# HugoZHL/MEVI

Measured on AMD Instinct MI355X. Metric: queries/sec @ MRR@10-match, MSMARCO dev, 1/2/4/8 MI355X, higher is better.
Workload: dtype f16+f32; 1 GPU; C2 dense arm (faiss_search.py Flat): 6980 x 768 f32 queries x 8841823 x 768 f32 docs, exact inner-product top-1000; queries=6980, docs=8841823, dim=768, topk=1000, parallelism=single GPU

## Files before the change

mevi_amd/csrc/ip_topk.hip:

```cpp

#include "mfma_pp_f16x16.h"

#include <float.h>
#include <math.h>
#include <string.h>
#include <vector>

namespace mevi {
namespace {

constexpr int MAX_SORT = 16384;

struct TopkGeom {
  int k;
  int S;
  int cap;
};

static inline int next_pow2(int x) {
  int p = 1;
  while (p < x) p <<= 1;
  return p;
}

// ... 465 lines not shown
  }
  __syncthreads();
}

__global__ __launch_bounds__(256) void compact_kernel(unsigned long long *__restrict__ buf,
                                                     unsigned int *__restrict__ count,
                                                     float *__restrict__ tau,
                                                     unsigned int *__restrict__ failed, int nq, int S, int k,
                                                     int cap) {
  extern __shared__ __attribute__((aligned(16))) unsigned long long skeys[];
  unsigned int *hist = reinterpret_cast<unsigned int *>(skeys + S);
  for (int q = blockIdx.x; q < nq; q += gridDim.x)
    compact_query(skeys, hist, buf + (size_t)q * S, count, tau, failed, q, k, cap);
}

template <int KPL>
__global__ __launch_bounds__(256) void compact_wave_kernel(unsigned long long *__restrict__ buf, unsigned int *__restrict__ count,
                                                          float *__restrict__ tau, unsigned int *__restrict__ failed, int nq,
                                                          int S, int k, int cap) {
  const int lane = threadIdx.x & 63;
  const int q = blockIdx.x * 4 + (int)(threadIdx.x >> 6);
  if (q >= nq) return;
  const unsigned int c_raw = count[q];
  if (c_raw == 0u) return;
  const int c = c_raw > (unsigned int)cap ? cap : (int)c_raw;
  const int n = k + c;
  if (n > 64 * KPL) return;
  unsigned long long *row = buf + (size_t)q * S;
  unsigned long long key[KPL];
#pragma unroll
  for (int j = 0; j < KPL; ++j) key[j] = (64 * j + lane < n) ? row[64 * j + lane] : 0ull;
  const int nj = (n + 63) >> 6;
  unsigned long long T = 0ull;
  bool exact = false;
  for (int b = 63; b >= 0; --b) {
    const unsigned long long cand = T | (1ull << b);
    int cnt = 0;
#pragma unroll
    for (int jb = 0; jb < KPL / 8; ++jb)
      if (8 * jb < nj) {
#pragma unroll
        for (int jj = 0; jj < 8; ++jj) cnt += __popcll(__ballot(key[8 * jb + jj] >= cand));
      }
    if (cnt >= k) {
      T = cand;
      if (cnt == k) {
        exact = true;
        break;
      }
    }
  }
  if (exact) {
    unsigned long long mn = ~0ull;
#pragma unroll
    for (int jb = 0; jb < KPL / 8; ++jb)
      if (8 * jb < nj) {
#pragma unroll
        for (int jj = 0; jj < 8; ++jj) {
          const unsigned long long kk = key[8 * jb + jj];
          if (kk >= T && kk < mn) mn = kk;
        }
      }
#pragma unroll
    for (int off = 32; off > 0; off >>= 1) {
      const unsigned long long o = ((unsigned long long)(unsigned int)__shfl_xor((int)(mn >> 32), off) << 32) |
                                   (unsigned int)__shfl_xor((int)mn, off);
      mn = o < mn ? o : mn;
    }
    T = mn;
  }
  int base = 0;
#pragma unroll
  for (int jb = 0; jb < KPL / 8; ++jb)
    if (8 * jb < nj) {
#pragma unroll
      for (int jj = 0; jj < 8; ++jj) {
        const unsigned long long kk = key[8 * jb + jj];
        const bool pass = kk > T;
        const unsigned long long mask = __ballot(pass);
        if (pass)
          row[base + (int)__builtin_amdgcn_mbcnt_hi((unsigned int)(mask >> 32), __builtin_amdgcn_mbcnt_lo((unsigned int)mask, 0u))] = kk;
        base += __popcll(mask);
      }
    }
  for (int i = base + lane; i < k; i += 64) row[i] = (i == k - 1) ? T : 0ull;
  if (lane == 0) {
    tau[q] = (T != 0ull) ? key_score(T) : -INFINITY;
    count[q] = 0u;
    if (c_raw > (unsigned int)cap) failed[q] = 1u;
  }
}

template <int KPL>
__global__ __launch_bounds__(256) void rank_tau_kernel(const unsigned long long *__restrict__ buf, int nq, int S, int k, int rank,
                                                      float *__restrict__ tau, float *__restrict__ tau_s) {
  const int lane = threadIdx.x & 63;
  const int q = blockIdx.x * 4 + (int)(threadIdx.x >> 6);
  if (q >= nq) return;
  const unsigned long long *row = buf + (size_t)q * S;
  unsigned long long key[KPL];
#pragma unroll
  for (int j = 0; j < KPL; ++j) key[j] = (64 * j + lane < k) ? row[64 * j + lane] : 0ull;
  const int nj = (k + 63) >> 6;
  unsigned long long T = 0ull;
// ... 851 lines not shown
      acc[1][0][r] = -INFINITY;
    }
    emit_tile<1>(acc, tq, 0, doc_begin + blk * 256 + 32 * w8, doc_end, buf, count, S, k, cap, id_base, stash);
    if (!have_nxt) break;
    blk = blk_n;
    cur = nxt;
    blk_n += gridDim.x;
    have_nxt = blk_n < n_blocks;
    if (have_nxt) nxt = src_of(blk_n);
  }
  asm volatile("s_waitcnt vmcnt(0)" ::: "memory");
  stash_flush(stash, buf, count, S, k, cap);
}

constexpr int RS_LD = 36;
__global__ __launch_bounds__(256) void rescore_rows_kernel(const float *__restrict__ Q, const float *__restrict__ D,
                                                          int dim, unsigned long long *__restrict__ buf, int S,
                                                          int kp, int nq, unsigned int id_base,
                                                          const float *__restrict__ qnorm,
                                                          const float *__restrict__ qinv,
                                                          const double *__restrict__ qshift, float c1, float c2,
                                                          const unsigned int *__restrict__ dmax_bits,
                                                          const float *__restrict__ dnorm_c,
                                                          unsigned int *__restrict__ err_ratio_bits,
                                                          const float *__restrict__ qdelta, const float *__restrict__ qn16,
                                                          const float *__restrict__ acc_k, int upper_keys = 0) {
  __shared__ __attribute__((aligned(16))) float tiles[4][64 * RS_LD];
  const int lane = threadIdx.x & 63;
  const int wave = __builtin_amdgcn_readfirstlane(threadIdx.x >> 6);
  const int wpq = (kp + 63) / 64;
  const long long gw = (long long)blockIdx.x * 4 + wave;
  const int q = (int)(gw / wpq);
  if (q >= nq) return;
  const int c = (int)(gw - (long long)q * wpq) * 64 + lane;
  unsigned long long *row = buf + (size_t)q * S;
  unsigned long long key = (c < kp) ? row[c] : 0ull;
  if (acc_k && key != 0ull) {
    const unsigned int idc = key_id(key) - id_base;
    const double e_max = h1_err_bound(qdelta[q], qn16[q], (double)__uint_as_float(dmax_bits[0]), (double)__uint_as_float(dmax_bits[3]), c1) +
                         (double)qnorm[q] * (double)c2 * __uint_as_float(dmax_bits[1]);
    const double e_c = h1_err_bound(qdelta[q], qn16[q], (double)dnorm_c[idc], (double)__uint_as_float(dmax_bits[3]), c1) +
                       (double)qnorm[q] * (double)c2 * __uint_as_float(dmax_bits[1]);
    if ((double)key_score(key) * (double)qinv[q] + e_c < (double)acc_k[q] * (double)qinv[q] - e_max) {
      key = 0ull;
      if (c < kp) row[c] = 0ull;
    }
  }
  const bool valid = key != 0ull;
  const unsigned int my_id = valid ? key_id(key) - id_base : 0u;
  float *sd = tiles[wave];
  const float *src[8];
#pragma unroll
  for (int i = 0; i < 8; ++i) src[i] = D + (size_t)__shfl(my_id, (lane >> 3) + 8 * i) * dim + (lane & 7) * 4;
  const float *qr = Q + (size_t)q * dim;
  const int nslab = (dim + 31) / 32;
  float4 v[8];
  auto fetch = [&](int s) {
    const bool in = s * 32 + (lane & 7) * 4 < dim;
#pragma unroll
    for (int i = 0; i < 8; ++i) v[i] = in ? *reinterpret_cast<const float4 *>(src[i] + s * 32) : make_float4(0.f, 0.f, 0.f, 0.f);
  };
  fetch(0);
  float acc = 0.f;
  for (int s = 0; s < nslab; ++s) {
#pragma unroll
    for (int i = 0; i < 8; ++i) *reinterpret_cast<float4 *>(sd + ((lane >> 3) + 8 * i) * RS_LD + (lane & 7) * 4) = v[i];
    if (s + 1 < nslab) fetch(s + 1);
    __builtin_amdgcn_wave_barrier();
    const float *dr = sd + lane * RS_LD;
#pragma unroll
    for (int k4 = 0; k4 < 32; k4 += 4) {
      const float4 x = *reinterpret_cast<const float4 *>(dr + k4);
      const int kk = s * 32 + k4;
      const float4 qq = kk < dim ? *reinterpret_cast<const float4 *>(qr + kk) : make_float4(0.f, 0.f, 0.f, 0.f);
      acc = fmaf(qq.x, x.x, acc);
      acc = fmaf(qq.y, x.y, acc);
      acc = fmaf(qq.z, x.z, acc);
      acc = fmaf(qq.w, x.w, acc);
    }
    __builtin_amdgcn_wave_barrier();
  }
  if (c < kp) row[c] = valid ? make_key(acc, key_id(key)) : 0ull;
  if (err_ratio_bits) {
    float ratio = 0.f;
    if (valid) {
      const double den = h1_err_bound(qdelta[q], qn16[q], (double)dnorm_c[my_id], (double)__uint_as_float(dmax_bits[3]), c1) +
                         (double)qnorm[q] * (double)c2 * __uint_as_float(dmax_bits[1]);
      const double est = (double)key_score(key) * (double)qinv[q] + qshift[q];
      if (den > 0.0) ratio = (float)((upper_keys ? fmax((double)acc - est, 0.0) : fabs(est - (double)acc)) / den);
    }
#pragma unroll
    for (int off = 32; off > 0; off >>= 1) ratio = fmaxf(ratio, __shfl_xor(ratio, off));
    if (lane == 0 && ratio > 0.f) atomicMax(err_ratio_bits, __float_as_uint(ratio));
  }
}

__global__ __launch_bounds__(256) void rescore_finish_kernel(const unsigned long long *__restrict__ buf, int S, int k,
                                                            int kp, const float *__restrict__ tau,
                                                            const float *__restrict__ qnorm,
                                                            const float *__restrict__ qinv,
                                                            const double *__restrict__ qshift, float c1, float c2,
                                                            const unsigned int *__restrict__ dmax_bits,
                                                            unsigned int *__restrict__ failed,
                                                            unsigned long long *__restrict__ out_top, int out_ld,
                                                            const float *__restrict__ qdelta, const float *__restrict__ qn16) {
  extern __shared__ __attribute__((aligned(16))) unsigned long long skeys[];
  const int q = blockIdx.x, t = threadIdx.x;
  int P = 64;
  while (P < kp) P <<= 1;
  const unsigned long long *row = buf + (size_t)q * S;
  for (int i = t; i < P; i += 256) skeys[i] = (i < kp) ? row[i] : 0ull;
  __syncthreads();
  bitonic_sort_desc<256>(skeys, P, t);
  for (int i = t; i < k; i += 256) out_top[(size_t)q * out_ld + i] = skeys[i];
  if (t == 0) {
    bool ok = true;
    const float a_last = tau[q];
    const double eps = h1_err_bound(qdelta[q], qn16[q], (double)__uint_as_float(dmax_bits[0]), (double)__uint_as_float(dmax_bits[3]), c1) +
                       (double)qnorm[q] * (double)c2 * __uint_as_float(dmax_bits[1]);
    if (a_last > -INFINITY) {
      const unsigned long long kth = skeys[k - 1];
      ok = (kth != 0ull) && ((double)a_last * (double)qinv[q] + qshift[q] + eps < (double)key_score(kth));
    }
    if (!(eps < 1.0e38)) ok = false;
    if (!ok) failed[q] = 1u;
  }
}

__global__ __launch_bounds__(256) void count_candidates_kernel(const unsigned int *__restrict__ count, int nq, int cap,
                                                              unsigned long long *__restrict__ out) {
  const int q = blockIdx.x * 256 + threadIdx.x;
  const unsigned int c = q < nq ? count[q] : 0u;
  unsigned long long sum = c;
  unsigned int mx = c, over = c > (unsigned int)cap ? 1u : 0u;
#pragma unroll
  for (int off = 32; off > 0; off >>= 1) {
    sum += ((unsigned long long)(unsigned int)__shfl_xor((int)(sum >> 32), off) << 32) | (unsigned int)__shfl_xor((int)sum, off);
    mx = max(mx, (unsigned int)__shfl_xor((int)mx, off));
    over += (unsigned int)__shfl_xor((int)over, off);
  }
// ... 38 lines not shown

struct ExactWs {
  SearchState st, fb;
  float *qsub; int *fidx;
  char *spare;
};
static ExactWs carve_exact(Carver &c, int64_t nq, int64_t dim, const TopkGeom &g) {
  return {carve_state(c, nq, g), carve_state(c, nq, g), c.take<float>((size_t)nq * dim), c.take<int>(nq), c.take<char>(256)};
}

struct QuerySide {
  float *image;
  float *norm, *inv, *delta, *n16;
  double *shift;
  unsigned int *err_bits;
};
static QuerySide carve_query_side(Carver &c, int64_t nq, size_t image_bytes) {
  QuerySide s = {reinterpret_cast<float *>(c.take<char>(image_bytes)), c.take<float>(nq + 1), c.take<float>(nq + 1),
                 c.take<float>(nq + 1), c.take<float>(nq + 1), c.take<double>(nq), nullptr};
  if (s.norm) s.err_bits = reinterpret_cast<unsigned int *>(s.norm + nq);
  return s;
}

thread_local double g_growth = 0.0;
thread_local int g_profile = 0;
thread_local mevi_ip_topk_stats g_stats = {0, 0, 0, 0.0, 0.0, 0.0, 0.0, 0.0, 0, 0, 0, 0};
thread_local std::vector<hipEvent_t> g_events;
thread_local std::vector<long long> g_chunk_rows;

static void profile_mark(hipStream_t stream) {
  if (!g_profile) return;
  hipEvent_t e;
  if (hipEventCreate(&e) != hipSuccess) return;
  (void)hipEventRecord(e, stream);
  g_events.push_back(e);
// ... 11 lines not shown
  }
  g_chunk_rows.clear();
  for (hipEvent_t e : g_events) (void)hipEventDestroy(e);
  g_events.clear();
}

enum class PassKind { ExactF32, F16Image, I8Image };
struct PassArgs {
  PassKind kind;
  const float *Q; int64_t nq;
  const float *D; int64_t nd; int dim;
  TopkGeom g; uint32_t id_base; SearchState st;
  bool guaranteed;
  unsigned long long *cand = nullptr;
  const float *row_scale = nullptr, *qub = nullptr;
};

enum class FilterGrid { PerTile, PerCU, SmallStream };
struct FilterChoice {
  const void *fn;
  size_t lds;
  int qt, ni16;
  FilterGrid grid;
};

static bool choose_filter(PassKind kind, int64_t nq, int dim, FilterChoice &f) {
  const bool h1 = kind != PassKind::ExactF32;
  const int ni = 2;
  static const bool shape32_f = [] { const char *e = getenv("MEVI_IP_FILTER_MFMA"); return e && atoi(e) == 32; }();
  static const int qt_pin = [] { const char *e = getenv("MEVI_IP_FILTER_QT"); return e ? atoi(e) : 0; }();
// ... 92 lines not shown
  const bool sample_on = sample_mode == 1 || (sample_mode != 0 && nq <= 1024);
  double s_c = 0.0;
  int64_t n_sample = 0;
  bool sampled = false;
  if (sample_on && !guaranteed && g.k <= 4096 && g.k >= 32) {
    const double r = g.k / 2 < 16 ? 16.0 : (g.k / 2 > 96 ? 96.0 : (double)(g.k / 2));
    double c = r >= 96.0 ? 3.0 : 8.0;
    const double c_fit = (double)g.cap / ((double)g.k * (1.0 + 8.0 / sqrt(r)));
    if (c_fit < c) c = c_fit;
    if (c >= 1.5 && (1.0 - 1.0 / c) * sqrt(r) >= 4.5) {
      s_c = c;
      n_sample = (int64_t)ceil(r * (double)nd / (c * (double)g.k));
    }
  }
  int64_t seen = 0, launches = 0;
  while (seen < nd) {
    int64_t chunk = cap_docs;
    if (!guaranteed && seen >= g.k) {
      int64_t grown = (int64_t)((double)seen * growth);
      grown = grown / (2 * BM) * (2 * BM);
      if (grown > chunk) chunk = grown;
    }
    if (chunk > nd - seen) chunk = nd - seen;
    double expect_per_q = seen >= g.k ? (double)g.k * (double)chunk / (double)seen : (double)chunk;
    if (s_c > 0.0 && !sampled && seen >= n_sample && seen >= g.k && chunk < nd - seen) {
      const int64_t rank = (int64_t)ceil(s_c * (double)g.k * (double)seen / (double)nd);
      if (rank >= 16 && rank <= g.k) {
        hipLaunchKernelGGL(rank_tau_kernel<64>, dim3((unsigned)((nq + 3) / 4)), dim3(256), 0, stream, st.buf, (int)nq, g.S, g.k, (int)rank,
                           st.tau, st.tau_s);
        sampled = true;
// ... 38 lines not shown
        flush_mask = T - 1;
        args[15] = &flush_mask;
        args[16] = (void *)&tickets;
        args[17] = (void *)&tickets_next;
      }
      if (hipLaunchKernel(f.fn, dim3(grid), dim3(PP_THREADS), args, f.lds, stream) != hipSuccess) {
        set_error("ip_topk: filter kernel launch failed");
        return -1;
      }
    }
    profile_mark(stream);
    if (a.cand)
      hipLaunchKernelGGL(count_candidates_kernel, dim3((unsigned)((nq + 255) / 256)), dim3(256), 0, stream, st.count, (int)nq, g.cap, a.cand);
    {
      const int nq_i = (int)nq;
      static const bool wave_compact = [] { const char *e = getenv("MEVI_IP_TOPK_COMPACT"); return !(e && strcmp(e, "lds") == 0); }();
      if (wave_compact)
        hipLaunchKernelGGL(compact_wave_kernel<64>, dim3((unsigned)((nq + 3) / 4)), dim3(256), 0, stream, st.buf, st.count, st.tau,
                           st.failed, nq_i, g.S, g.k, g.cap);
      hipLaunchKernelGGL(compact_kernel, dim3((unsigned)(nq < 8 * n_cu ? nq : 8 * n_cu)), dim3(256), compact_lds, stream,
                         st.buf, st.count, st.tau, st.failed, nq_i, g.S, g.k, g.cap);
    }
    if (sampled && seen + chunk >= nd)
      hipLaunchKernelGGL(sample_check_kernel, dim3((unsigned)((nq + 255) / 256)), dim3(256), 0, stream, st.tau, st.tau_s, st.failed, (int)nq);
    profile_mark(stream);
    g_stats.filter_flops += 2.0 * (double)nq * (double)chunk * (double)a.dim;
    if (g_profile) g_chunk_rows.push_back((long long)chunk);
    seen += chunk;
    ++launches;
  }
  if (a.kind == PassKind::ExactF32)
    hipLaunchKernelGGL(sort_lists_kernel, dim3((unsigned)nq), dim3(256), (size_t)next_pow2(g.k < 64 ? 64 : g.k) * 8, stream,
                       st.buf, g.S, g.k);
  if (hipGetLastError() != hipSuccess) {
    set_error("ip_topk: kernel launch failed");
    return -1;
  }
  return launches;
}

static void finalize(const unsigned long long *lists, int ld, int64_t k, int64_t nq, float *out_score, int64_t *out_id, hipStream_t stream) {
  hipLaunchKernelGGL(finalize_kernel, dim3((unsigned)((nq * (long long)k + 255) / 256)), dim3(256), 0, stream, lists, ld, (int)k,
                     (long long)nq, out_score, reinterpret_cast<long long *>(out_id));
}

// ... 192 lines not shown
  IndexedWs w = {};
  w.first = carve_f16_pass(c, nq, dim, k, make_geom(h1_kprime((int)k), nq));
  if (const int kp2 = h1_kprime2((int)k)) {
    const int64_t n2 = h1_second_pass_max(nq);
    w.second = carve_f16_pass(c, n2, dim, k, make_geom(kp2));
    w.q2 = c.take<float>((size_t)n2 * dim);
    w.idx2 = c.take<int>(n2);
  }
  w.exact = carve_exact(c, nq, dim, make_geom((int)k));
  w.counters = c.take<unsigned long long>(32);
  return w;
}

void prove(const float *q, const float *docs, int64_t nq, int64_t dim, int64_t k, const TopkGeom &gp, uint32_t id_base,
           const SearchState &st, const QuerySide &qs, unsigned long long *top, float c1, float c2, const unsigned int *bits,
           const float *dnorms, unsigned int *err_bits, const float *acc_k, int upper_keys, hipStream_t stream) {
  const int kp = gp.k, P = next_pow2(kp < 64 ? 64 : kp);
  const long long waves = nq * (long long)((kp + 63) / 64);
  hipLaunchKernelGGL(rescore_rows_kernel, dim3((unsigned)((waves + 3) / 4)), dim3(256), 0, stream, q, docs, (int)dim, st.buf,
                     gp.S, kp, (int)nq, (unsigned int)id_base, qs.norm, qs.inv, qs.shift, c1, c2, bits, dnorms, err_bits, qs.delta,
                     qs.n16, acc_k, upper_keys);
  hipLaunchKernelGGL(rescore_finish_kernel, dim3((unsigned)nq), dim3(256), (size_t)P * 8, stream, st.buf, gp.S, (int)k, kp,
                     st.tau, qs.norm, qs.inv, qs.shift, c1, c2, bits, st.failed, top, (int)k, qs.delta, qs.n16);
}
}

extern "C" size_t mevi_ip_topk_indexed_workspace_bytes(int64_t nq, int64_t dim, int64_t k) {
  if (nq <= 0 || k <= 0 || k > 4096 || dim <= 0) return 0;
  return carved_bytes([&](Carver &c) { carve_indexed(c, nq, dim, k); });
}

extern "C" int mevi_ip_topk_indexed_f32(const float *q, int64_t nq, const float *docs, const void *index, int64_t nd,
                                        int64_t dim, int64_t k, int64_t id_offset, float *out_score,
                                        int64_t *out_id, void *workspace, size_t workspace_bytes, void *stream_) {
  hipStream_t stream = reinterpret_cast<hipStream_t>(stream_);
  begin_call();
  if (const int rc = check_search("ip_topk_indexed", true, q, nq, docs, index, nd, dim, k, id_offset, out_score, out_id, workspace,
                                  workspace_bytes, mevi_ip_topk_indexed_workspace_bytes(nq, dim, k)))
// ... 4 lines not shown
  const TopkGeom gp = make_geom(kp, nq), g = make_geom((int)k);
  const int64_t dimp = pad_k(dim);
  IndexView iv = view_index(index, nd, dim);
  Carver carver(workspace);
  const IndexedWs w = carve_indexed(carver, nq, dim, k);
  const SearchState &st = w.first.st;
  const QuerySide &qs = w.first.qs;
  unsigned long long *const top = w.first.top;
  const float c1 = h1_cacc(dimp), c2 = h1_c2(dim);
  unsigned long long *cand = g_profile >= 2 ? w.counters : nullptr;
  if (cand) MEVI_HIP_CHECK(hipMemsetAsync(cand, 0, 32, stream));

  hipLaunchKernelGGL(split_queries_f16_kernel, dim3((unsigned)(image_rows(nq) / 4)), dim3(256), 0, stream, q, (long long)nq,
                     (int)dim, (int)dimp, iv.mu, iv.scal, reinterpret_cast<_Float16 *>(qs.image), qs.norm, qs.inv, qs.shift, qs.delta,
                     qs.n16);
  int64_t launches = run_pass({PassKind::F16Image, qs.image, nq, iv.image, nd, (int)dimp, gp, (uint32_t)id_offset, st, false, cand}, stream);
  if (launches < 0) return MEVI_ERR_HIP;
  g_stats.n_chunks = launches;
  g_stats.filter_flops *= (double)dim / (double)dimp;
  MEVI_HIP_CHECK(hipMemsetAsync(qs.err_bits, 0, 4, stream));
  {
    static const bool rescore_all = [] { const char *e = getenv("MEVI_IP_RESCORE_ALL"); return e && atoi(e) == 1; }();
    const float *acc_k = nullptr;
    if (!rescore_all && kp <= 4096 && k < kp) {
      hipLaunchKernelGGL(rank_tau_kernel<64>, dim3((unsigned)((nq + 3) / 4)), dim3(256), 0, stream, st.buf, (int)nq, gp.S, kp, (int)k,
                         (float *)nullptr, st.tau_s);
      acc_k = st.tau_s;
    }
    prove(q, docs, nq, dim, k, gp, (uint32_t)id_offset, st, qs, top, c1, c2, iv.bits, iv.norms_c, qs.err_bits, acc_k, 0, stream);
  }
  finalize(top, (int)k, k, nq, out_score, out_id, stream);
  float err_ratio = 0.f;
  MEVI_HIP_CHECK(hipMemcpyAsync(&err_ratio, qs.err_bits, 4, hipMemcpyDeviceToHost, stream));
  unsigned long long cand_host[3] = {0ull, 0ull, 0ull};
  if (cand) MEVI_HIP_CHECK(hipMemcpyAsync(cand_host, cand, 24, hipMemcpyDeviceToHost, stream));
  MEVI_HIP_CHECK(hipGetLastError());
  std::vector<unsigned int> failed((size_t)nq);
  MEVI_HIP_CHECK(hipMemcpyAsync(failed.data(), st.failed, (size_t)nq * 4, hipMemcpyDeviceToHost, stream));
  MEVI_HIP_CHECK(hipStreamSynchronize(stream));
  profile_collect();
  g_stats.max_err_ratio = err_ratio;
  g_stats.err_bound = 1.0;
  g_stats.n_filter_candidates = (int64_t)cand_host[0];
  g_stats.max_launch_candidates = (int64_t)cand_host[1];
  g_stats.n_list_overflows = (int64_t)cand_host[2];
  const bool bound_suspect = g_stats.max_err_ratio > 1.0;
  std::vector<int> idx;
  for (int64_t i = 0; i < nq; ++i)
    if (failed[(size_t)i] || bound_suspect) idx.push_back((int)i);
  const bool repaired = !idx.empty();
  const int kp2 = h1_kprime2((int)k);
  if (!idx.empty() && !bound_suspect && kp2 != 0 && (int64_t)idx.size() <= h1_second_pass_max(nq)) {
    const int64_t n2 = (int64_t)idx.size();
    g_stats.n_second_pass_queries = n2;
    const TopkGeom g2 = make_geom(kp2);
    const SearchState &s2 = w.second.st;
    const QuerySide &qs2 = w.second.qs;
    MEVI_HIP_CHECK(hipMemcpyAsync(w.idx2, idx.data(), (size_t)n2 * 4, hipMemcpyHostToDevice, stream));
    hipLaunchKernelGGL(gather_rows_kernel, dim3((unsigned)n2), dim3(256), 0, stream, q, w.idx2, (int)n2, (int)dim, w.q2);
    hipLaunchKernelGGL(split_queries_f16_kernel, dim3((unsigned)(image_rows(n2) / 4)), dim3(256), 0, stream, w.q2, (long long)n2,
                       (int)dim, (int)dimp, iv.mu, iv.scal, reinterpret_cast<_Float16 *>(qs2.image), qs2.norm, qs2.inv, qs2.shift,
                       qs2.delta, qs2.n16);
    const double keep_flops = g_stats.filter_flops;
    const int64_t l2 = run_pass({PassKind::F16Image, qs2.image, n2, iv.image, nd, (int)dimp, g2, (uint32_t)id_offset, s2, false}, stream);
    g_stats.filter_flops = keep_flops;
    if (l2 < 0) return MEVI_ERR_HIP;
    prove(w.q2, docs, n2, dim, k, g2, (uint32_t)id_offset, s2, qs2, w.second.top, c1, c2, iv.bits, iv.norms_c, nullptr, nullptr, 0,
          stream);
    hipLaunchKernelGGL(scatter_top_kernel, dim3((unsigned)n2), dim3(256), 0, stream, w.second.top, w.idx2, (int)n2, (int)k, (int)k, top,
                       (int)k);
    std::vector<unsigned int> failed2((size_t)n2);
    MEVI_HIP_CHECK(hipMemcpyAsync(failed2.data(), s2.failed, (size_t)n2 * 4, hipMemcpyDeviceToHost, stream));
    MEVI_HIP_CHECK(hipStreamSynchronize(stream));
    profile_collect();
    std::vector<int> still;
    for (int64_t i = 0; i < n2; ++i)
      if (failed2[(size_t)i]) still.push_back(idx[(size_t)i]);
    idx.swap(still);
  }
  if (!idx.empty())
    if (const int rc = exact_repair(q, idx, docs, nd, (int)dim, g, (uint32_t)id_offset, w.exact, top, (int)k, true, stream)) return rc;
  if (repaired) finalize(top, (int)k, k, nq, out_score, out_id, stream);
  MEVI_HIP_CHECK(hipGetLastError());
  return MEVI_OK;
}

namespace {
struct Index8View {
// ... 103 lines not shown
  const int64_t dimp = pad_k(dim);
  const IndexView iv = view_index(index, nd, dim);
  const Index8View v8 = view_index8(index8, nd, dim);
  Carver carver(workspace);
  const I8Pass w = carve_i8_pass(carver, nq, dim, k);
  const SearchState &st = w.p.st;
  const QuerySide &qs = w.p.qs;
  const float c1 = (float)(1.001 / 4194304.0), c2 = h1_c2(dim);

  hipLaunchKernelGGL(split_queries_i8_kernel, dim3(8), dim3(256), 0, stream, q, (int)nq, (int)dim, (int)dimp, iv.mu, v8.cscale,
                     reinterpret_cast<signed char *>(qs.image), qs.norm, qs.inv, qs.shift, qs.delta, qs.n16, v8.bits, w.qub, w.qbad);
  const int64_t launches = run_pass({PassKind::I8Image, qs.image, nq, v8.image, nd, (int)dimp, gp, (uint32_t)id_offset, st, false, nullptr,
                                     v8.scale, w.qub}, stream);
  if (launches < 0) return MEVI_ERR_HIP;
  MEVI_HIP_CHECK(hipMemsetAsync(qs.err_bits, 0, 4, stream));
  prove(q, docs, nq, dim, k, gp, (uint32_t)id_offset, st, qs, w.p.top, c1, c2, v8.bits, v8.ynorm, qs.err_bits, nullptr, 1, stream);
  finalize(w.p.top, (int)k, k, nq, out_score, out_id, stream);
  float ratio = 0.f;
  MEVI_HIP_CHECK(hipMemcpyAsync(&ratio, qs.err_bits, 4, hipMemcpyDeviceToHost, stream));
  MEVI_HIP_CHECK(hipGetLastError());
  unsigned int failed[32], bad[32];
  MEVI_HIP_CHECK(hipMemcpyAsync(failed, st.failed, (size_t)nq * 4, hipMemcpyDeviceToHost, stream));
  MEVI_HIP_CHECK(hipMemcpyAsync(bad, w.qbad, (size_t)nq * 4, hipMemcpyDeviceToHost, stream));
  MEVI_HIP_CHECK(hipStreamSynchronize(stream));
  profile_collect();
  int64_t open = 0;
  for (int64_t i = 0; i < nq; ++i) open += (failed[i] || bad[i]) ? 1 : 0;
  if (!(ratio <= 1.0f)) open = nq;
  g_stats.n_chunks = launches;
  g_stats.max_err_ratio = ratio;
  g_stats.err_bound = 1.0;
  g_stats.n_i8_queries = nq;
// ... 69 lines not shown
```

Before: 82680 queries/s.

## Fuse rescore, finish and finalize into one prove kernel; fold rank tau into compaction

Merges the separate rescore-rows, rescore-finish and finalize launches into a single prove_kernel that splits each query's candidates over G blocks and prefetches the next key group's documents. The wave-level compaction now streams candidates in register-sized windows, uses a 32-bit high-word radix search with min/max prefix narrowing, and computes the rank-k threshold in the same pass, so the standalone rank_tau launch is avoided. The host reads a single fail word before copying the per-query failure array. This is meant to cut launch count, repeated threshold searches and D2H traffic, at the cost of more complex, register-heavy kernels and a new dependence on the fused kernel's cross-block correctness.

Measured after the change: 82780 queries/s (median of 6 runs). About the same (+0.1%).

```diff
diff --git a/mevi_amd/csrc/ip_topk.hip b/mevi_amd/csrc/ip_topk.hip
--- a/mevi_amd/csrc/ip_topk.hip
+++ b/mevi_amd/csrc/ip_topk.hip
@@ -503,80 +503,167 @@
     compact_query(skeys, hist, buf + (size_t)q * S, count, tau, failed, q, k, cap);
 }
 
+constexpr int COMPACT_KPL = 64;
 template <int KPL>
 __global__ __launch_bounds__(256) void compact_wave_kernel(unsigned long long *__restrict__ buf, unsigned int *__restrict__ count,
                                                           float *__restrict__ tau, unsigned int *__restrict__ failed, int nq,
-                                                          int S, int k, int cap) {
+                                                          int S, int k, int cap, int rank, float *__restrict__ tau_s) {
   const int lane = threadIdx.x & 63;
   const int q = blockIdx.x * 4 + (int)(threadIdx.x >> 6);
   if (q >= nq) return;
   const unsigned int c_raw = count[q];
-  if (c_raw == 0u) return;
+  if (c_raw == 0u && rank == 0) return;
   const int c = c_raw > (unsigned int)cap ? cap : (int)c_raw;
-  const int n = k + c;
-  if (n > 64 * KPL) return;
+  const int kreg = (k + 63) >> 6;
+  const int room = 64 * (KPL - kreg);
   unsigned long long *row = buf + (size_t)q * S;
   unsigned long long key[KPL];
-#pragma unroll
-  for (int j = 0; j < KPL; ++j) key[j] = (64 * j + lane < n) ? row[64 * j + lane] : 0ull;
-  const int nj = (n + 63) >> 6;
-  unsigned long long T = 0ull;
-  bool exact = false;
-  for (int b = 63; b >= 0; --b) {
-    const unsigned long long cand = T | (1ull << b);
+  int nj = 0;
+  auto count_ge = [&](unsigned int cand) {
     int cnt = 0;
 #pragma unroll
     for (int jb = 0; jb < KPL / 8; ++jb)
       if (8 * jb < nj) {
 #pragma unroll
-        for (int jj = 0; jj < 8; ++jj) cnt += __popcll(__ballot(key[8 * jb + jj] >= cand));
+        for (int jj = 0; jj < 8; ++jj) cnt += __popcll(__ballot((unsigned int)(key[8 * jb + jj] >> 32) >= cand));
       }
-    if (cnt >= k) {
-      T = cand;
-      if (cnt == k) {
-        exact = true;
-        break;
-      }
-    }
-  }
-  if (exact) {
-    unsigned long long mn = ~0ull;
+    return cnt;
+  };
+  unsigned long long T = 0ull;
+  unsigned int pre = 0u;
+  int pre_bit = 31, nz = 0;
+  int done = 0;
+  do {
+    const int take = c - done < room ? c - done : room;
+    const int shift = k + done - 64 * kreg;
+    nj = kreg + ((take + 63) >> 6);
+    int k_r = k, kreg_r = kreg, lane_r = lane;
+    asm volatile("" : "+s"(k_r), "+s"(kreg_r), "+v"(lane_r));
 #pragma unroll
     for (int jb = 0; jb < KPL / 8; ++jb)
       if (8 * jb < nj) {
 #pragma unroll
         for (int jj = 0; jj < 8; ++jj) {
-          const unsigned long long kk = key[8 * jb + jj];
-          if (kk >= T && kk < mn) mn = kk;
+          const int j = 8 * jb + jj, i = 64 * j + lane_r;
+          const bool lst = j < kreg_r;
+          const bool in = lst ? i < k_r : i - 64 * kreg_r < take;
+          const unsigned long long e = row[in ? i + (lst ? 0 : shift) : 0];
+          key[j] = in ? e : 0ull;
+        }
+      } else {
+#pragma unroll
+        for (int jj = 0; jj < 8; ++jj) key[8 * jb + jj] = 0ull;
+      }
+    unsigned int mn1 = ~0u, mx = 0u;
+    nz = 0;
+#pragma unroll
+    for (int jb = 0; jb < KPL / 8; ++jb)
+      if (8 * jb < nj) {
+#pragma unroll
+        for (int jj = 0; jj < 8; ++jj) {
+          const unsigned int h = (unsigned int)(key[8 * jb + jj] >> 32);
+          nz += __popcll(__ballot(h != 0u));
+          mn1 = min(mn1, h - 1u);
+          mx = max(mx, h);
         }
       }
 #pragma unroll
     for (int off = 32; off > 0; off >>= 1) {
-      const unsigned long long o = ((unsigned long long)(unsigned int)__shfl_xor((int)(mn >> 32), off) << 32) |
-                                   (unsigned int)__shfl_xor((int)mn, off);
-      mn = o < mn ? o : mn;
-    }
-    T = mn;
-  }
-  int base = 0;
-#pragma unroll
-  for (int jb = 0; jb < KPL / 8; ++jb)
-    if (8 * jb < nj) {
-#pragma unroll
-      for (int jj = 0; jj < 8; ++jj) {
-        const unsigned long long kk = key[8 * jb + jj];
-        const bool pass = kk > T;
-        const unsigned long long mask = __ballot(pass);
-        if (pass)
-          row[base + (int)__builtin_amdgcn_mbcnt_hi((unsigned int)(mask >> 32), __builtin_amdgcn_mbcnt_lo((unsigned int)mask, 0u))] = kk;
-        base += __popcll(mask);
+      mn1 = min(mn1, (unsigned int)__shfl_xor((int)mn1, off));
+      mx = max(mx, (unsigned int)__shfl_xor((int)mx, off));
+    }
+    mn1 = (unsigned int)__builtin_amdgcn_readfirstlane((int)mn1);
+    mx = (unsigned int)__builtin_amdgcn_readfirstlane((int)mx);
+    T = 0ull;
+    if (nz >= k) {
+      const unsigned int diff = (mn1 + 1u) ^ mx;
+      pre_bit = diff ? 31 - __clz((int)diff) : -1;
+      pre = pre_bit >= 31 ? 0u : (pre_bit < 0 ? mx : (mx >> (pre_bit + 1)) << (pre_bit + 1));
+      unsigned int Th = pre;
+      bool exact = nz == k;
+      for (int b = pre_bit; b >= 0 && !exact; --b) {
+        const unsigned int cand = Th | (1u << b);
+        const int cnt = count_ge(cand);
+        if (cnt >= k) {
+          Th = cand;
+          exact = cnt == k;
+        }
       }
-    }
-  for (int i = base + lane; i < k; i += 64) row[i] = (i == k - 1) ? T : 0ull;
+      if (exact) {
+        unsigned long long mn = ~0ull;
+        const unsigned int floor_h = Th ? Th : 1u;
+#pragma unroll
+        for (int jb = 0; jb < KPL / 8; ++jb)
+          if (8 * jb < nj) {
+#pragma unroll
+            for (int jj = 0; jj < 8; ++jj) {
+              const unsigned long long kk = key[8 * jb + jj];
+              if ((unsigned int)(kk >> 32) >= floor_h && kk < mn) mn = kk;
+            }
+          }
+#pragma unroll
+        for (int off = 32; off > 0; off >>= 1) {
+          const unsigned long long o = ((unsigned long long)(unsigned int)__shfl_xor((int)(mn >> 32), off) << 32) |
+                                       (unsigned int)__shfl_xor((int)mn, off);
+          mn = o < mn ? o : mn;
+        }
+        T = mn;
+      } else {
+        const int need = k - (Th == ~0u ? 0 : count_ge(Th + 1u));
+        unsigned int Tl = 0u;
+        for (int b = 31; b >= 0; --b) {
+          const unsigned int cand = Tl | (1u << b);
+          unsigned int th_r = Th;
+          asm volatile("" : "+v"(th_r));
+          int cnt = 0;
+#pragma unroll
+          for (int jb = 0; jb < KPL / 8; ++jb)
+            if (8 * jb < nj) {
+#pragma unroll
+              for (int jj = 0; jj < 8; ++jj) {
+                const unsigned long long kk = key[8 * jb + jj];
+                cnt += __popcll(__ballot((unsigned int)(kk >> 32) == th_r && (unsigned int)kk >= cand));
+              }
+            }
+          if (cnt >= need) Tl = cand;
+        }
+        T = ((unsigned long long)Th << 32) | (unsigned long long)Tl;
+      }
+    }
+    int base = 0;
+#pragma unroll
+    for (int jb = 0; jb < KPL / 8; ++jb)
+      if (8 * jb < nj) {
+#pragma unroll
+        for (int jj = 0; jj < 8; ++jj) {
+          const unsigned long long kk = key[8 * jb + jj];
+          const bool pass = kk > T;
+          const unsigned long long mask = __ballot(pass);
+          if (pass)
+            row[base + (int)__builtin_amdgcn_mbcnt_hi((unsigned int)(mask >> 32), __builtin_amdgcn_mbcnt_lo((unsigned int)mask, 0u))] = kk;
+          base += __popcll(mask);
+        }
+      }
+    for (int i = base + lane; i < k; i += 64) row[i] = (i == k - 1) ? T : 0ull;
+    done += take;
+    if (done < c) __threadfence_block();
+  } while (done < c);
+  float ts = -INFINITY;
+  if (rank > 0 && nz >= rank) {
+    unsigned int Tr = nz >= k ? pre : 0u;
+    for (int b = nz >= k ? pre_bit : 31; b >= 0; --b) {
+      const unsigned int cand = Tr | (1u << b);
+      if (count_ge(cand) >= rank) Tr = cand;
+    }
+    ts = ord_to_f32(Tr);
+  }
   if (lane == 0) {
-    tau[q] = (T != 0ull) ? key_score(T) : -INFINITY;
-    count[q] = 0u;
-    if (c_raw > (unsigned int)cap) failed[q] = 1u;
+    if (c_raw != 0u) {
+      tau[q] = (T != 0ull) ? key_score(T) : -INFINITY;
+      count[q] = 0u;
+      if (c_raw > (unsigned int)cap) failed[q] = 1u;
+    }
+    if (rank > 0) tau_s[q] = ts;
   }
 }
 
@@ -1458,116 +1545,151 @@
 }
 
 constexpr int RS_LD = 36;
-__global__ __launch_bounds__(256) void rescore_rows_kernel(const float *__restrict__ Q, const float *__restrict__ D,
-                                                          int dim, unsigned long long *__restrict__ buf, int S,
-                                                          int kp, int nq, unsigned int id_base,
-                                                          const float *__restrict__ qnorm,
-                                                          const float *__restrict__ qinv,
-                                                          const double *__restrict__ qshift, float c1, float c2,
-                                                          const unsigned int *__restrict__ dmax_bits,
-                                                          const float *__restrict__ dnorm_c,
-                                                          unsigned int *__restrict__ err_ratio_bits,
-                                                          const float *__restrict__ qdelta, const float *__restrict__ qn16,
-                                                          const float *__restrict__ acc_k, int upper_keys = 0) {
-  __shared__ __attribute__((aligned(16))) float tiles[4][64 * RS_LD];
-  const int lane = threadIdx.x & 63;
-  const int wave = __builtin_amdgcn_readfirstlane(threadIdx.x >> 6);
+constexpr size_t PROVE_TILE_BYTES = (size_t)4 * 64 * RS_LD * 4;
+__global__ __launch_bounds__(256) void prove_kernel(const float *__restrict__ Q, const float *__restrict__ D, int dim,
+                                                   unsigned long long *buf, int S, int k, int kp, int G, unsigned int id_base,
+                                                   unsigned int *__restrict__ count, const float *__restrict__ tau,
+                                                   const float *__restrict__ qnorm, const float *__restrict__ qinv,
+                                                   const double *__restrict__ qshift, float c1, float c2,
+                                                   const unsigned int *__restrict__ dmax_bits, const float *__restrict__ dnorm_c,
+                                                   unsigned int *__restrict__ err_ratio_bits, const float *__restrict__ qdelta,
+                                                   const float *__restrict__ qn16, const float *__restrict__ acc_k, int upper_keys,
+                                                   unsigned int *__restrict__ failed, unsigned int *__restrict__ fail_word,
+                                                   unsigned long long *__restrict__ out_top, float *__restrict__ out_score,
+                                                   long long *__restrict__ out_id) {
+  extern __shared__ __attribute__((aligned(16))) unsigned long long skeys[];
+  const int t = threadIdx.x, lane = t & 63;
+  const int wave = __builtin_amdgcn_readfirstlane(t >> 6);
+  const int q = (int)(blockIdx.x / (unsigned int)G), g = (int)(blockIdx.x - (unsigned int)q * (unsigned int)G);
   const int wpq = (kp + 63) / 64;
-  const long long gw = (long long)blockIdx.x * 4 + wave;
-  const int q = (int)(gw / wpq);
-  if (q >= nq) return;
-  const int c = (int)(gw - (long long)q * wpq) * 64 + lane;
   unsigned long long *row = buf + (size_t)q * S;
-  unsigned long long key = (c < kp) ? row[c] : 0ull;
-  if (acc_k && key != 0ull) {
-    const unsigned int idc = key_id(key) - id_base;
-    const double e_max = h1_err_bound(qdelta[q], qn16[q], (double)__uint_as_float(dmax_bits[0]), (double)__uint_as_float(dmax_bits[3]), c1) +
-                         (double)qnorm[q] * (double)c2 * __uint_as_float(dmax_bits[1]);
-    const double e_c = h1_err_bound(qdelta[q], qn16[q], (double)dnorm_c[idc], (double)__uint_as_float(dmax_bits[3]), c1) +
-                       (double)qnorm[q] * (double)c2 * __uint_as_float(dmax_bits[1]);
-    if ((double)key_score(key) * (double)qinv[q] + e_c < (double)acc_k[q] * (double)qinv[q] - e_max) {
-      key = 0ull;
-      if (c < kp) row[c] = 0ull;
-    }
-  }
-  const bool valid = key != 0ull;
-  const unsigned int my_id = valid ? key_id(key) - id_base : 0u;
-  float *sd = tiles[wave];
-  const float *src[8];
-#pragma unroll
-  for (int i = 0; i < 8; ++i) src[i] = D + (size_t)__shfl(my_id, (lane >> 3) + 8 * i) * dim + (lane & 7) * 4;
+  float *sd = reinterpret_cast<float *>(skeys) + wave * (64 * RS_LD);
   const float *qr = Q + (size_t)q * dim;
   const int nslab = (dim + 31) / 32;
+  const double e_q = (double)qnorm[q] * (double)c2 * __uint_as_float(dmax_bits[1]);
+  auto load_key = [&](int grp) {
+    const int c = grp * 64 + lane;
+    unsigned long long key = (c < kp) ? row[c] : 0ull;
+    if (acc_k && key != 0ull) {
+      const unsigned int idc = key_id(key) - id_base;
+      const double e_max = h1_err_bound(qdelta[q], qn16[q], (double)__uint_as_float(dmax_bits[0]), (double)__uint_as_float(dmax_bits[3]), c1) + e_q;
+      const double e_c = h1_err_bound(qdelta[q], qn16[q], (double)dnorm_c[idc], (double)__uint_as_float(dmax_bits[3]), c1) + e_q;
+      if ((double)key_score(key) * (double)qinv[q] + e_c < (double)acc_k[q] * (double)qinv[q] - e_max) {
+        key = 0ull;
+        row[c] = 0ull;
+      }
+    }
+    return key;
+  };
+  const float *src[8];
+  auto set_src = [&](unsigned long long key) {
+    const unsigned int id = key != 0ull ? key_id(key) - id_base : 0u;
+#pragma unroll
+    for (int i = 0; i < 8; ++i) src[i] = D + (size_t)__shfl(id, (lane >> 3) + 8 * i) * dim + (lane & 7) * 4;
+  };
   float4 v[8];
   auto fetch = [&](int s) {
     const bool in = s * 32 + (lane & 7) * 4 < dim;
 #pragma unroll
     for (int i = 0; i < 8; ++i) v[i] = in ? *reinterpret_cast<const float4 *>(src[i] + s * 32) : make_float4(0.f, 0.f, 0.f, 0.f);
   };
-  fetch(0);
-  float acc = 0.f;
-  for (int s = 0; s < nslab; ++s) {
-#pragma unroll
-    for (int i = 0; i < 8; ++i) *reinterpret_cast<float4 *>(sd + ((lane >> 3) + 8 * i) * RS_LD + (lane & 7) * 4) = v[i];
-    if (s + 1 < nslab) fetch(s + 1);
-    __builtin_amdgcn_wave_barrier();
-    const float *dr = sd + lane * RS_LD;
-#pragma unroll
-    for (int k4 = 0; k4 < 32; k4 += 4) {
-      const float4 x = *reinterpret_cast<const float4 *>(dr + k4);
-      const int kk = s * 32 + k4;
-      const float4 qq = kk < dim ? *reinterpret_cast<const float4 *>(qr + kk) : make_float4(0.f, 0.f, 0.f, 0.f);
-      acc = fmaf(qq.x, x.x, acc);
-      acc = fmaf(qq.y, x.y, acc);
-      acc = fmaf(qq.z, x.z, acc);
-      acc = fmaf(qq.w, x.w, acc);
-    }
-    __builtin_amdgcn_wave_barrier();
-  }
-  if (c < kp) row[c] = valid ? make_key(acc, key_id(key)) : 0ull;
+  const int step = 4 * G;
+  int grp = 4 * g + wave;
+  unsigned long long key = 0ull;
+  if (grp < wpq) {
+    key = load_key(grp);
+    set_src(key);
+    fetch(0);
+  }
+  float ratio = 0.f;
+  for (; grp < wpq; grp += step) {
+    const bool more = grp + step < wpq;
+    const unsigned long long key_n = more ? load_key(grp + step) : 0ull;
+    float acc = 0.f;
+    for (int s = 0; s < nslab; ++s) {
+#pragma unroll
+      for (int i = 0; i < 8; ++i) *reinterpret_cast<float4 *>(sd + ((lane >> 3) + 8 * i) * RS_LD + (lane & 7) * 4) = v[i];
+      if (s + 1 < nslab) {
+        fetch(s + 1);
+      } else if (more) {
+        set_src(key_n);
+        fetch(0);
+      }
+      __builtin_amdgcn_wave_barrier();
+      const float *dr = sd + lane * RS_LD;
+#pragma unroll
+      for (int k4 = 0; k4 < 32; k4 += 4) {
+        const float4 x = *reinterpret_cast<const float4 *>(dr + k4);
+        const int kk = s * 32 + k4;
+        const float4 qq = kk < dim ? *reinterpret_cast<const float4 *>(qr + kk) : make_float4(0.f, 0.f, 0.f, 0.f);
+        acc = fmaf(qq.x, x.x, acc);
+        acc = fmaf(qq.y, x.y, acc);
+        acc = fmaf(qq.z, x.z, acc);
+        acc = fmaf(qq.w, x.w, acc);
+      }
+      __builtin_amdgcn_wave_barrier();
+    }
+    const bool valid = key != 0ull;
+    const int c = grp * 64 + lane;
+    if (c < kp) row[c] = valid ? make_key(acc, key_id(key)) : 0ull;
+    if (err_ratio_bits && valid) {
+      const double den = h1_err_bound(qdelta[q], qn16[q], (double)dnorm_c[key_id(key) - id_base], (double)__uint_as_float(dmax_bits[3]), c1) + e_q;
+      const double est = (double)key_score(key) * (double)qinv[q] + qshift[q];
+      if (den > 0.0) ratio = fmaxf(ratio, (float)((upper_keys ? fmax((double)acc - est, 0.0) : fabs(est - (double)acc)) / den));
+    }
+    key = key_n;
+  }
   if (err_ratio_bits) {
-    float ratio = 0.f;
-    if (valid) {
-      const double den = h1_err_bound(qdelta[q], qn16[q], (double)dnorm_c[my_id], (double)__uint_as_float(dmax_bits[3]), c1) +
-                         (double)qnorm[q] * (double)c2 * __uint_as_float(dmax_bits[1]);
-      const double est = (double)key_score(key) * (double)qinv[q] + qshift[q];
-      if (den > 0.0) ratio = (float)((upper_keys ? fmax((double)acc - est, 0.0) : fabs(est - (double)acc)) / den);
-    }
 #pragma unroll
     for (int off = 32; off > 0; off >>= 1) ratio = fmaxf(ratio, __shfl_xor(ratio, off));
     if (lane == 0 && ratio > 0.f) atomicMax(err_ratio_bits, __float_as_uint(ratio));
   }
-}
-
-__global__ __launch_bounds__(256) void rescore_finish_kernel(const unsigned long long *__restrict__ buf, int S, int k,
-                                                            int kp, const float *__restrict__ tau,
-                                                            const float *__restrict__ qnorm,
-                                                            const float *__restrict__ qinv,
-                                                            const double *__restrict__ qshift, float c1, float c2,
-                                                            const unsigned int *__restrict__ dmax_bits,
-                                                            unsigned int *__restrict__ failed,
-                                                            unsigned long long *__restrict__ out_top, int out_ld,
-                                                            const float *__restrict__ qdelta, const float *__restrict__ qn16) {
-  extern __shared__ __attribute__((aligned(16))) unsigned long long skeys[];
-  const int q = blockIdx.x, t = threadIdx.x;
+  asm volatile("s_waitcnt vmcnt(0)" ::: "memory");
+  __syncthreads();
+  if (G > 1) {
+    unsigned int *flag = reinterpret_cast<unsigned int *>(skeys);
+    if (t == 0) {
+      __builtin_amdgcn_fence(__ATOMIC_RELEASE, "agent");
+      asm volatile("s_waitcnt vmcnt(0)" ::: "memory");
+      const unsigned int arrived = __hip_atomic_fetch_add(&count[q], 1u, __ATOMIC_RELAXED, __HIP_MEMORY_SCOPE_AGENT);
+      const bool last = arrived == (unsigned int)(G - 1);
+      if (last) {
+        __builtin_amdgcn_fence(__ATOMIC_ACQUIRE, "agent");
+        asm volatile("s_waitcnt vmcnt(0)" ::: "memory");
+        count[q] = 0u;
+      }
+      *flag = last ? 1u : 0u;
+    }
+    __syncthreads();
+    const bool last = *flag != 0u;
+    __syncthreads();
+    if (!last) return;
+  }
   int P = 64;
   while (P < kp) P <<= 1;
-  const unsigned long long *row = buf + (size_t)q * S;
   for (int i = t; i < P; i += 256) skeys[i] = (i < kp) ? row[i] : 0ull;
   __syncthreads();
   bitonic_sort_desc<256>(skeys, P, t);
-  for (int i = t; i < k; i += 256) out_top[(size_t)q * out_ld + i] = skeys[i];
+  for (int i = t; i < k; i += 256) {
+    const unsigned long long e = skeys[i];
+    const size_t o = (size_t)q * k + i;
+    out_top[o] = e;
+    if (out_score) {
+      out_score[o] = e == 0ull ? -FLT_MAX : key_score(e);
+      out_id[o] = e == 0ull ? -1ll : (long long)key_id(e);
+    }
+  }
   if (t == 0) {
     bool ok = true;
     const float a_last = tau[q];
-    const double eps = h1_err_bound(qdelta[q], qn16[q], (double)__uint_as_float(dmax_bits[0]), (double)__uint_as_float(dmax_bits[3]), c1) +
-                       (double)qnorm[q] * (double)c2 * __uint_as_float(dmax_bits[1]);
+    const double eps = h1_err_bound(qdelta[q], qn16[q], (double)__uint_as_float(dmax_bits[0]), (double)__uint_as_float(dmax_bits[3]), c1) + e_q;
     if (a_last > -INFINITY) {
       const unsigned long long kth = skeys[k - 1];
       ok = (kth != 0ull) && ((double)a_last * (double)qinv[q] + qshift[q] + eps < (double)key_score(kth));
     }
     if (!(eps < 1.0e38)) ok = false;
     if (!ok) failed[q] = 1u;
+    if (fail_word && (!ok || failed[q] != 0u)) atomicOr(fail_word, 1u);
   }
 }
 
@@ -1636,11 +1758,13 @@
   float *norm, *inv, *delta, *n16;
   double *shift;
   unsigned int *err_bits;
+  unsigned int *fail_word;
 };
 static QuerySide carve_query_side(Carver &c, int64_t nq, size_t image_bytes) {
   QuerySide s = {reinterpret_cast<float *>(c.take<char>(image_bytes)), c.take<float>(nq + 1), c.take<float>(nq + 1),
-                 c.take<float>(nq + 1), c.take<float>(nq + 1), c.take<double>(nq), nullptr};
+                 c.take<float>(nq + 1), c.take<float>(nq + 1), c.take<double>(nq), nullptr, nullptr};
   if (s.norm) s.err_bits = reinterpret_cast<unsigned int *>(s.norm + nq);
+  if (s.inv) s.fail_word = reinterpret_cast<unsigned int *>(s.inv + nq);
   return s;
 }
 
@@ -1682,6 +1806,7 @@
   bool guaranteed;
   unsigned long long *cand = nullptr;
   const float *row_scale = nullptr, *qub = nullptr;
+  int rank_k = 0;
 };
 
 enum class FilterGrid { PerTile, PerCU, SmallStream };
@@ -1804,6 +1929,7 @@
     }
   }
   int64_t seen = 0, launches = 0;
+  bool ranked = false;
   while (seen < nd) {
     int64_t chunk = cap_docs;
     if (!guaranteed && seen >= g.k) {
@@ -1872,12 +1998,16 @@
       hipLaunchKernelGGL(count_candidates_kernel, dim3((unsigned)((nq + 255) / 256)), dim3(256), 0, stream, st.count, (int)nq, g.cap, a.cand);
     {
       const int nq_i = (int)nq;
-      static const bool wave_compact = [] { const char *e = getenv("MEVI_IP_TOPK_COMPACT"); return !(e && strcmp(e, "lds") == 0); }();
-      if (wave_compact)
-        hipLaunchKernelGGL(compact_wave_kernel<64>, dim3((unsigned)((nq + 3) / 4)), dim3(256), 0, stream, st.buf, st.count, st.tau,
-                           st.failed, nq_i, g.S, g.k, g.cap);
-      hipLaunchKernelGGL(compact_kernel, dim3((unsigned)(nq < 8 * n_cu ? nq : 8 * n_cu)), dim3(256), compact_lds, stream,
-                         st.buf, st.count, st.tau, st.failed, nq_i, g.S, g.k, g.cap);
+      static const bool lds_pinned = [] { const char *e = getenv("MEVI_IP_TOPK_COMPACT"); return e && strcmp(e, "lds") == 0; }();
+      if (!lds_pinned && g.k <= 64 * COMPACT_KPL - 1024) {
+        const int rank = (a.rank_k > 0 && seen + chunk >= nd && !sampled) ? a.rank_k : 0;
+        hipLaunchKernelGGL(compact_wave_kernel<COMPACT_KPL>, dim3((unsigned)((nq + 3) / 4)), dim3(256), 0, stream, st.buf, st.count,
+                           st.tau, st.failed, nq_i, g.S, g.k, g.cap, rank, st.tau_s);
+        if (rank) ranked = true;
+      } else {
+        hipLaunchKernelGGL(compact_kernel, dim3((unsigned)(nq < 8 * n_cu ? nq : 8 * n_cu)), dim3(256), compact_lds, stream,
+                           st.buf, st.count, st.tau, st.failed, nq_i, g.S, g.k, g.cap);
+      }
     }
     if (sampled && seen + chunk >= nd)
       hipLaunchKernelGGL(sample_check_kernel, dim3((unsigned)((nq + 255) / 256)), dim3(256), 0, stream, st.tau, st.tau_s, st.failed, (int)nq);
@@ -1887,6 +2017,9 @@
     seen += chunk;
     ++launches;
   }
+  if (a.rank_k > 0 && !ranked)
+    hipLaunchKernelGGL(rank_tau_kernel<64>, dim3((unsigned)((nq + 3) / 4)), dim3(256), 0, stream, st.buf, (int)nq, g.S, g.k, a.rank_k,
+                       (float *)nullptr, st.tau_s);
   if (a.kind == PassKind::ExactF32)
     hipLaunchKernelGGL(sort_lists_kernel, dim3((unsigned)nq), dim3(256), (size_t)next_pow2(g.k < 64 ? 64 : g.k) * 8, stream,
                        st.buf, g.S, g.k);
@@ -2109,14 +2242,24 @@
 
 void prove(const float *q, const float *docs, int64_t nq, int64_t dim, int64_t k, const TopkGeom &gp, uint32_t id_base,
            const SearchState &st, const QuerySide &qs, unsigned long long *top, float c1, float c2, const unsigned int *bits,
-           const float *dnorms, unsigned int *err_bits, const float *acc_k, int upper_keys, hipStream_t stream) {
+           const float *dnorms, unsigned int *err_bits, const float *acc_k, int upper_keys, bool summary, float *out_score,
+           int64_t *out_id, hipStream_t stream) {
   const int kp = gp.k, P = next_pow2(kp < 64 ? 64 : kp);
-  const long long waves = nq * (long long)((kp + 63) / 64);
-  hipLaunchKernelGGL(rescore_rows_kernel, dim3((unsigned)((waves + 3) / 4)), dim3(256), 0, stream, q, docs, (int)dim, st.buf,
-                     gp.S, kp, (int)nq, (unsigned int)id_base, qs.norm, qs.inv, qs.shift, c1, c2, bits, dnorms, err_bits, qs.delta,
-                     qs.n16, acc_k, upper_keys);
-  hipLaunchKernelGGL(rescore_finish_kernel, dim3((unsigned)nq), dim3(256), (size_t)P * 8, stream, st.buf, gp.S, (int)k, kp,
-                     st.tau, qs.norm, qs.inv, qs.shift, c1, c2, bits, st.failed, top, (int)k, qs.delta, qs.n16);
+  int n_cu = 256;
+  {
+    int dev = 0, v = 0;
+    if (hipGetDevice(&dev) == hipSuccess && hipDeviceGetAttribute(&v, hipDeviceAttributeMultiprocessorCount, dev) == hipSuccess && v >= 8)
+      n_cu = v;
+  }
+  const int64_t wpq = (kp + 63) / 64;
+  int64_t G = (4 * (int64_t)n_cu + nq - 1) / nq;
+  if (G > (wpq + 3) / 4) G = (wpq + 3) / 4;
+  if (G < 1) G = 1;
+  const size_t lds = (size_t)P * 8 > PROVE_TILE_BYTES ? (size_t)P * 8 : PROVE_TILE_BYTES;
+  hipLaunchKernelGGL(prove_kernel, dim3((unsigned)(nq * G)), dim3(256), lds, stream, q, docs, (int)dim, st.buf, gp.S, (int)k, kp,
+                     (int)G, (unsigned int)id_base, st.count, st.tau, qs.norm, qs.inv, qs.shift, c1, c2, bits, dnorms, err_bits,
+                     qs.delta, qs.n16, acc_k, upper_keys, st.failed, summary ? qs.fail_word : (unsigned int *)nullptr, top, out_score,
+                     reinterpret_cast<long long *>(out_id));
 }
 }
 
@@ -2151,30 +2294,31 @@
   hipLaunchKernelGGL(split_queries_f16_kernel, dim3((unsigned)(image_rows(nq) / 4)), dim3(256), 0, stream, q, (long long)nq,
                      (int)dim, (int)dimp, iv.mu, iv.scal, reinterpret_cast<_Float16 *>(qs.image), qs.norm, qs.inv, qs.shift, qs.delta,
                      qs.n16);
-  int64_t launches = run_pass({PassKind::F16Image, qs.image, nq, iv.image, nd, (int)dimp, gp, (uint32_t)id_offset, st, false, cand}, stream);
+  MEVI_HIP_CHECK(hipMemsetAsync(qs.err_bits, 0, 4, stream));
+  MEVI_HIP_CHECK(hipMemsetAsync(qs.fail_word, 0, 4, stream));
+  static const bool rescore_all = [] { const char *e = getenv("MEVI_IP_RESCORE_ALL"); return e && atoi(e) == 1; }();
+  const bool exclude = !rescore_all && kp <= 4096 && k < kp;
+  PassArgs pass = {PassKind::F16Image, qs.image, nq, iv.image, nd, (int)dimp, gp, (uint32_t)id_offset, st, false, cand};
+  pass.rank_k = exclude ? (int)k : 0;
+  int64_t launches = run_pass(pass, stream);
   if (launches < 0) return MEVI_ERR_HIP;
   g_stats.n_chunks = launches;
   g_stats.filter_flops *= (double)dim / (double)dimp;
-  MEVI_HIP_CHECK(hipMemsetAsync(qs.err_bits, 0, 4, stream));
-  {
-    static const bool rescore_all = [] { const char *e = getenv("MEVI_IP_RESCORE_ALL"); return e && atoi(e) == 1; }();
-    const float *acc_k = nullptr;
-    if (!rescore_all && kp <= 4096 && k < kp) {
-      hipLaunchKernelGGL(rank_tau_kernel<64>, dim3((unsigned)((nq + 3) / 4)), dim3(256), 0, stream, st.buf, (int)nq, gp.S, kp, (int)k,
-                         (float *)nullptr, st.tau_s);
-      acc_k = st.tau_s;
-    }
-    prove(q, docs, nq, dim, k, gp, (uint32_t)id_offset, st, qs, top, c1, c2, iv.bits, iv.norms_c, qs.err_bits, acc_k, 0, stream);
-  }
-  finalize(top, (int)k, k, nq, out_score, out_id, stream);
+  prove(q, docs, nq, dim, k, gp, (uint32_t)id_offset, st, qs, top, c1, c2, iv.bits, iv.norms_c, qs.err_bits, exclude ? st.tau_s : nullptr,
+        0, true, out_score, out_id, stream);
   float err_ratio = 0.f;
+  unsigned int any_failed = 0u;
   MEVI_HIP_CHECK(hipMemcpyAsync(&err_ratio, qs.err_bits, 4, hipMemcpyDeviceToHost, stream));
+  MEVI_HIP_CHECK(hipMemcpyAsync(&any_failed, qs.fail_word, 4, hipMemcpyDeviceToHost, stream));
   unsigned long long cand_host[3] = {0ull, 0ull, 0ull};
   if (cand) MEVI_HIP_CHECK(hipMemcpyAsync(cand_host, cand, 24, hipMemcpyDeviceToHost, stream));
   MEVI_HIP_CHECK(hipGetLastError());
+  MEVI_HIP_CHECK(hipStreamSynchronize(stream));
   std::vector<unsigned int> failed((size_t)nq);
-  MEVI_HIP_CHECK(hipMemcpyAsync(failed.data(), st.failed, (size_t)nq * 4, hipMemcpyDeviceToHost, stream));
-  MEVI_HIP_CHECK(hipStreamSynchronize(stream));
+  if (any_failed) {
+    MEVI_HIP_CHECK(hipMemcpyAsync(failed.data(), st.failed, (size_t)nq * 4, hipMemcpyDeviceToHost, stream));
+    MEVI_HIP_CHECK(hipStreamSynchronize(stream));
+  }
   profile_collect();
   g_stats.max_err_ratio = err_ratio;
   g_stats.err_bound = 1.0;
@@ -2198,17 +2342,23 @@
     hipLaunchKernelGGL(split_queries_f16_kernel, dim3((unsigned)(image_rows(n2) / 4)), dim3(256), 0, stream, w.q2, (long long)n2,
                        (int)dim, (int)dimp, iv.mu, iv.scal, reinterpret_cast<_Float16 *>(qs2.image), qs2.norm, qs2.inv, qs2.shift,
                        qs2.delta, qs2.n16);
+    MEVI_HIP_CHECK(hipMemsetAsync(qs2.fail_word, 0, 4, stream));
     const double keep_flops = g_stats.filter_flops;
     const int64_t l2 = run_pass({PassKind::F16Image, qs2.image, n2, iv.image, nd, (int)dimp, g2, (uint32_t)id_offset, s2, false}, stream);
     g_stats.filter_flops = keep_flops;
     if (l2 < 0) return MEVI_ERR_HIP;
     prove(w.q2, docs, n2, dim, k, g2, (uint32_t)id_offset, s2, qs2, w.second.top, c1, c2, iv.bits, iv.norms_c, nullptr, nullptr, 0,
-          stream);
+          true, nullptr, nullptr, stream);
     hipLaunchKernelGGL(scatter_top_kernel, dim3((unsigned)n2), dim3(256), 0, stream, w.second.top, w.idx2, (int)n2, (int)k, (int)k, top,
                        (int)k);
     std::vector<unsigned int> failed2((size_t)n2);
-    MEVI_HIP_CHECK(hipMemcpyAsync(failed2.data(), s2.failed, (size_t)n2 * 4, hipMemcpyDeviceToHost, stream));
+    unsigned int any_failed2 = 0u;
+    MEVI_HIP_CHECK(hipMemcpyAsync(&any_failed2, qs2.fail_word, 4, hipMemcpyDeviceToHost, stream));
     MEVI_HIP_CHECK(hipStreamSynchronize(stream));
+    if (any_failed2) {
+      MEVI_HIP_CHECK(hipMemcpyAsync(failed2.data(), s2.failed, (size_t)n2 * 4, hipMemcpyDeviceToHost, stream));
+      MEVI_HIP_CHECK(hipStreamSynchronize(stream));
+    }
     profile_collect();
     std::vector<int> still;
     for (int64_t i = 0; i < n2; ++i)
@@ -2342,8 +2492,8 @@
                                      v8.scale, w.qub}, stream);
   if (launches < 0) return MEVI_ERR_HIP;
   MEVI_HIP_CHECK(hipMemsetAsync(qs.err_bits, 0, 4, stream));
-  prove(q, docs, nq, dim, k, gp, (uint32_t)id_offset, st, qs, w.p.top, c1, c2, v8.bits, v8.ynorm, qs.err_bits, nullptr, 1, stream);
-  finalize(w.p.top, (int)k, k, nq, out_score, out_id, stream);
+  prove(q, docs, nq, dim, k, gp, (uint32_t)id_offset, st, qs, w.p.top, c1, c2, v8.bits, v8.ynorm, qs.err_bits, nullptr, 1, false,
+        out_score, out_id, stream);
   float ratio = 0.f;
   MEVI_HIP_CHECK(hipMemcpyAsync(&ratio, qs.err_bits, 4, hipMemcpyDeviceToHost, stream));
   MEVI_HIP_CHECK(hipGetLastError());
```
